# eezkni/UEGAN

Hardware: AMD Instinct MI355X
Metric: train imgs/sec @512px bs=16 on 1/2/4/8 MI355X; infer ms/img (higher is better)
Workload: dtype bf16; 1 GPU; FiveK-shaped 512x512 batch=16/GPU, full G/D/VGG train step (trainer.py:77-119), conv_dim=32, seeded stand-in VGG19; global_batch=16, parallelism=dp1, pool_size=50, collective=none (1 rank), passes=batched (fused.py)

## Files before the change

### include/uegan_hip.h

```cpp
#ifndef UEGAN_HIP_H_
#define UEGAN_HIP_H_

#include <stddef.h>
#include <stdint.h>

#ifdef __cplusplus
extern "C" {
#endif

#define UEGAN_VERSION 105

enum { UEGAN_OK = 0, UEGAN_E_INVALID = -1, UEGAN_E_HIP = -2, UEGAN_E_UNSUPPORTED = -3 };
enum { UEGAN_F32 = 0, UEGAN_BF16 = 1 };
enum { UEGAN_PAD_ZERO = 0, UEGAN_PAD_REFLECT = 1 };
enum { UEGAN_ACT_NONE = 0, UEGAN_ACT_LRELU = 1, UEGAN_ACT_RELU = 2, UEGAN_ACT_TANH = 3,
       UEGAN_ACT_SIGMOID = 4,
       UEGAN_ACT_SWISH = 5, UEGAN_ACT_SELU = 6 };
enum { UEGAN_IMPL_AUTO = 0, UEGAN_IMPL_MFMA = 1, UEGAN_IMPL_DIRECT = 2, UEGAN_IMPL_MFMA_REGSTAGE = 3, UEGAN_IMPL_MFMA_GENERIC = 4 };

typedef void* uegan_stream_t;

int uegan_version(void);
const char* uegan_last_error(void);
int uegan_set_conv_impl(int impl);
enum {
  UEGAN_TUNE_SMALL_GRID = 0,
  UEGAN_TUNE_FOLD_MAX = 1,
  UEGAN_TUNE_HEADS_NO_CG = 2,
  UEGAN_TUNE_WIDE_MIN_GRID = 3,
  UEGAN_TUNE_TALL_MIN_GRID = 4,
  UEGAN_TUNE_TALL_RPW = 5,
  UEGAN_TUNE_TALL_REFLECT = 6,
  UEGAN_TUNE_FLAT_S2 = 7,
  UEGAN_TUNE_TOEP_HEADS = 8,
  UEGAN_TUNE_HEADS_MFMA = 9,
  UEGAN_TUNE_FWD_STATS = 10,
  UEGAN_TUNE_WGRAD_XCD = 11,
  UEGAN_TUNE_VGG_EPI = 12,
  UEGAN_TUNE_GAM_BWD = 13,
  UEGAN_TUNE_COUNT = 14
};
int uegan_set_tuning(int knob, int value, int* previous);
int uegan_selftest_mfma(void* scratch_4096_floats, uegan_stream_t stream);

typedef struct {
  char name[96];
  int64_t launches;
  double total_ms;
  double total_flops;
  double total_bytes;
} uegan_profile_entry;
int uegan_profile_begin(int max_records);
int uegan_profile_end(uegan_profile_entry* out, int max_entries, int* n_entries);

typedef struct {
  int32_t dtype;
  int32_t B, H, W;
  int32_t C1, C2;
  int32_t Ho, Wo, Cout;
  int32_t KH, KW, stride, pad;
  int32_t pad_mode;
  int32_t act;
  int32_t Cin_w, Cout_w;
  int32_t Cin_total;
  int32_t scale_group;
} uegan_conv_desc;

int64_t uegan_packed_k(int64_t k);
int uegan_pack_weights(int dtype, const float* w_oihw, int Cout, int Cin, int KH, int KW, int Cout_pad, int Cin_pad, void* w_ohwi,
                       void* w_ihwo, uegan_stream_t stream);
int uegan_pack_weights_slice(int dtype, const float* w_oihw, int Cout, int Cin, int Cin_total, int KH, int KW, int Cout_pad, int Cin_pad,
                             void* w_ohwi, void* w_ihwo, uegan_stream_t stream);
int uegan_pack_weights_pair(int dtype, const float* w_oihw, int Cout, int Cin, int Cin_total, int KH, int KW, int Cout_pad, int Cin_pad,
                            void* w_ohwi, void* w_ihwo, void* w_ohwi_lo, int dup_cin, uegan_stream_t stream);
typedef struct uegan_pack_entry {
  const float* w_oihw;
  void* w_ohwi;
  void* w_ihwo;
  int64_t start;
  int32_t Cout, Cin, Cin_total, KH, KW, Cout_pad, Cin_pad, Kp, Kp2;
  int32_t flags;
  void* w_ohwi_lo;
} uegan_pack_entry;
int uegan_pack_weights_multi(int dtype, const uegan_pack_entry* table_dev, int n_entries, int64_t total, uegan_stream_t stream);
int uegan_conv2d_fwd(const uegan_conv_desc* d, const void* x1, const void* x2, const void* w_ohwi, const float* bias,
                     const float* scale, void* y, uegan_stream_t stream);
size_t uegan_conv2d_fwd_splitk_workspace_bytes(const uegan_conv_desc* d);
int uegan_conv2d_fwd_splitk(const uegan_conv_desc* d, const void* x1, const void* x2, const void* w_ohwi, const float* bias, const float* scale, void* y,
                            void* workspace, size_t workspace_bytes, uegan_stream_t stream);
size_t uegan_conv2d_fwd_stats_workspace_bytes(const uegan_conv_desc* d);
int uegan_conv2d_fwd_stats(const uegan_conv_desc* d, const void* x1, const void* x2, const void* w_ohwi, const float* bias, const float* scale, void* y,
                           float* mean, float* rstd, float eps, void* workspace, size_t workspace_bytes, int* produced, uegan_stream_t stream);
int uegan_instnorm_apply(int dtype, const void* x, void* y, const float* mean, const float* rstd, int B, int HW, int C, uegan_stream_t stream);

typedef struct {
  const void* x1_lo;
  const void* x2_lo;
  const void* w_lo;
  void* y_lo;
  const void* mul;
  const void* mul_lo;
  void* y_mul;
  void* y_mul_lo;
  const float* res_x;
  const float* res_x2;
  float* res_out;
  float* res_out2;
  float* mean;
  float* rstd;
  void* stats_workspace;
  size_t stats_workspace_bytes;
  float eps;
  int32_t res_split;
  int32_t w_interleaved;
  int32_t reserved;
} uegan_conv_ex;
size_t uegan_conv2d_fwd_ex_workspace_bytes(const uegan_conv_desc* d, const uegan_conv_ex* ex);
int uegan_conv2d_fwd_ex(const uegan_conv_desc* d, const uegan_conv_ex* ex, const void* x1, const void* x2, const void* w_ohwi, const float* bias,
                        const float* scale, void* y, int* taken, uegan_stream_t stream);
int uegan_nchw_to_nhwc_pair(int dtype, const float* x, void* y, int B, int C, int Cp, int H, int W, const float* a, const float* b,
                            uegan_stream_t stream);
int uegan_instnorm_apply_pair(int dtype, const void* x, const void* x_lo, void* y, void* y_lo, const float* mean, const float* rstd, int B, int HW,
                              int C, uegan_stream_t stream);
// ... 210 lines not shown
```

### uegan_amd/csrc/conv_core.h

```cpp
#pragma once
#include "common.h"
#include "conv_internal.h"

#include <stdio.h>
#include <stdlib.h>
#include <utility>
#include <vector>

namespace uegan {

struct ProfRecord {
  hipEvent_t start, stop;
  int kernel_id;
  double flops, bytes;
};
extern bool g_prof_on;
extern std::vector<ProfRecord> g_prof_records;
extern std::vector<std::pair<hipEvent_t, hipEvent_t>> g_prof_pool;
extern size_t g_prof_used;

static inline int prof_key(int kind, bool bf16, int bn, int ks, int mode, int th, bool glds) {
  return (kind << 28) | ((bf16 ? 1 : 0) << 24) | (bn << 12) | (ks << 8) | (mode << 4) | ((th == 32 ? 2 : (th == 16 ? 1 : (th == 4 ? 3 : 0))) << 1) | (glds ? 1 : 0);
}
static void prof_kernel_name(int key, char* buf, size_t n) {
  const int kind = (key >> 28) & 7, bn = (key >> 12) & 0xfff, ks = (key >> 8) & 15, mode = (key >> 4) & 15;
  const char* dt = ((key >> 24) & 1) ? "bf16" : "f32";
  if (kind == 0) snprintf(buf, n, "conv_gemm_kernel<%s,BN=%d,%s>", dt, bn, (key & 1) ? "glds" : "regstage");
  else if (kind == 1) snprintf(buf, n, "conv_patch_kernel<%s,BN=%d,KS=%d,MODE=%d,TH=%d>", dt, bn, ks, mode, 8 << ((key >> 1) & 3));
  else if (kind == 4) snprintf(buf, n, "conv_stream_kernel<%s,TN=%d,PF=%d,MODE=%d>", dt, bn, ks, mode);
  else if (kind == 5) snprintf(buf, n, "conv_s2fwd_kernel<%s,BN=%d,K=%d,TH=%d>", dt, bn, ks, 8 << ((key >> 1) & 3));
  else if (kind == 6) snprintf(buf, n, "conv_toep_kernel<%s,K=%d,MODE=%d>", dt, ks, mode);
  else if (kind == 7 && ((key >> 1) & 3) == 1) snprintf(buf, n, "conv_tall_kernel<%s,BN=%d,KS=%d,MODE=%d%s>", dt, bn, ks, mode, (key & 1) ? "" : ",POOL");
  else if (kind == 7 && ((key >> 1) & 3) == 3) snprintf(buf, n, "conv_flat_kernel<%s,BN=%d,KS=%d>", dt, bn, ks);
  else if (kind == 7) snprintf(buf, n, "conv_wide_kernel<%s,BN=%d,KS=%d,MODE=%d>", dt, bn, ks, mode);
  else if (kind == 3) snprintf(buf, n, "wgrad_tr_kernel<%s,TN=%d,TM=%d%s>", dt, bn, ks, (key & 1) ? ",big" : "");
  else snprintf(buf, n, "conv_wgrad_kernel<%s,BN=%d>", dt, bn);
}

struct ProfScope {
  bool on;
  hipStream_t s;
  ProfRecord rec;
  ProfScope(int kernel_id, double flops, hipStream_t stream, double bytes = 0.0) : on(g_prof_on && g_prof_used < g_prof_pool.size()), s(stream) {
    if (!on) return;
    rec.bytes = bytes;
    rec.start = g_prof_pool[g_prof_used].first;
    rec.stop = g_prof_pool[g_prof_used].second;
    ++g_prof_used;
    rec.kernel_id = kernel_id;
    rec.flops = flops;
    (void)hipEventRecord(rec.start, s);
  }
  ~ProfScope() {
    if (!on) return;
    (void)hipEventRecord(rec.stop, s);
    g_prof_records.push_back(rec);
  }
};

#ifdef UEGAN_HALF_FP16
typedef _Float16 bf16x8_t __attribute__((ext_vector_type(8)));
__device__ __forceinline__ f32x4 mfma_bf16(u32x4 a, u32x4 b, f32x4 c) {
  return __builtin_amdgcn_mfma_f32_16x16x32_f16(__builtin_bit_cast(bf16x8_t, a), __builtin_bit_cast(bf16x8_t, b), c, 0, 0, 0);
}
#else
typedef __bf16 bf16x8_t __attribute__((ext_vector_type(8)));

__device__ __forceinline__ f32x4 mfma_bf16(u32x4 a, u32x4 b, f32x4 c) {
  return __builtin_amdgcn_mfma_f32_16x16x32_bf16(__builtin_bit_cast(bf16x8_t, a), __builtin_bit_cast(bf16x8_t, b), c, 0, 0, 0);
}
#endif
__device__ __forceinline__ f32x4 mfma_f32(float a, float b, f32x4 c) {
  return __builtin_amdgcn_mfma_f32_16x16x4f32(a, b, c, 0, 0, 0);
}

template <typename T> __device__ __forceinline__ u32x4 add_frag(u32x4 a, u32x4 b);
template <> __device__ __forceinline__ u32x4 add_frag<bf16_t>(u32x4 a, u32x4 b) {
  u32x4 r;
#pragma unroll
  for (int d = 0; d < 4; ++d) r[d] = pack_bf16x2(half_lo_to_f32(a[d]) + half_lo_to_f32(b[d]), half_hi_to_f32(a[d]) + half_hi_to_f32(b[d]));
  return r;
}
template <> __device__ __forceinline__ u32x4 add_frag<float>(u32x4 a, u32x4 b) {
  u32x4 r;
#pragma unroll
  for (int d = 0; d < 4; ++d) r[d] = f32_to_bits(bits_to_f32(a[d]) + bits_to_f32(b[d]));
  return r;
}

template <typename T> struct Mma;
template <> struct Mma<bf16_t> {
  static constexpr int NCHUNK = 1;
  static __device__ __forceinline__ void step(const u32x4* a, const u32x4* b, f32x4& acc) { acc = mfma_bf16(a[0], b[0], acc); }
};
template <> struct Mma<float> {
  static constexpr int NCHUNK = 2;
  static __device__ __forceinline__ void step(const u32x4* a, const u32x4* b, f32x4& acc) {
#pragma unroll
    for (int c = 0; c < 2; ++c) {
      acc = mfma_f32(bits_to_f32(a[c].x), bits_to_f32(b[c].x), acc);
      acc = mfma_f32(bits_to_f32(a[c].y), bits_to_f32(b[c].y), acc);
      acc = mfma_f32(bits_to_f32(a[c].z), bits_to_f32(b[c].z), acc);
      acc = mfma_f32(bits_to_f32(a[c].w), bits_to_f32(b[c].w), acc);
    }
  }
};

struct ConvGeom {
  int B, IH, IW;
  int C1, C2, C;
  int OH, OW;
  int KH, KW, stride, pad, pad_mode;
  int mode;
};

__device__ __forceinline__ int src_coord(const ConvGeom& g, int o, int t, int img, int in_n, int out_n) {
  if (g.mode == 0) {
// ... 86 lines not shown
  int N, Kp, act, nbias;
  int nty, ntx;
  int frame;
  int fy0, fy1, fx0, fx1;
  const void* mask;
  int mask_act;
  void* pool_out = nullptr;
  int pool_done = 0;
  void* pool_idx = nullptr;
  int n_idx = 0;
  int n_full = 1 << 30;
  int xcd_map = 0;
  int epi = 0;
  const void* epi_y = nullptr;
  const float* epi_st = nullptr;
  const float* epi_tot = nullptr;
  const float* epi_gscale = nullptr;
  float epi_weight = 0.f;
  const unsigned char* epi_idx = nullptr;
  int rect_y0 = 0, rect_y1 = 0, rect_x0 = 0, rect_x1 = 0;
  int border_only = 0;
  float* stats_part = nullptr;
  int stats_tpi = 0;
  const void* in1_lo = nullptr;
  const void* in2_lo = nullptr;
  const void* w_lo = nullptr;
  void* out_lo = nullptr;
  const void* mul = nullptr;
  const void* mul_lo = nullptr;
  void* out_mul = nullptr;
  void* out_mul_lo = nullptr;
  int src_wrap = 0;
  const float* res_x = nullptr;
  const float* res_x2 = nullptr;
  float* res_out = nullptr;
  float* res_out2 = nullptr;
  int res_split = 1 << 30;
  float* kws = nullptr;
  size_t kws_bytes = 0;
  int kparts = 0, kchunks = 0;
};

static inline int splitk_parts(const ConvArgs& a, int blocks, int nchunk, int* kchunks) {
  *kchunks = nchunk;
  if (!a.kws || a.g.mode != 0 || a.frame || a.out2 || a.mask || a.pool_out || a.stats_part || a.out_lo || a.mul || a.res_out || blocks <= 0) return 1;
  int parts = 1;
  while (parts * 2 <= nchunk && blocks * parts * 2 <= 256) parts *= 2;
  const size_t out_bytes = (size_t)a.g.B * a.g.OH * a.g.OW * a.N * sizeof(float);
  while (parts > 1 && (size_t)parts * out_bytes > a.kws_bytes) parts >>= 1;
  if (parts < 2) return 1;
  *kchunks = (nchunk + parts - 1) / parts;
  return (nchunk + *kchunks - 1) / *kchunks;
}

int splitk_reduce_launch(const ConvArgs& a, hipStream_t s);


constexpr int CONV_TH = 8, CONV_TW = 16, CONV_BM = CONV_TH * CONV_TW;
constexpr int CONV_ROWB = 128;

struct ConvImpl { int impl; bool glds, patch, heads, wgtr, stream; };
extern ConvImpl g_impl;

int check_desc(const uegan_conv_desc* d);
ConvGeom fwd_geom(const uegan_conv_desc* d);
static inline int cin_w(const uegan_conv_desc* d) { return d->Cin_w ? d->Cin_w : d->C1 + d->C2; }
static inline int cin_row(const uegan_conv_desc* d) { return d->Cin_total ? d->Cin_total : cin_w(d); }
static inline int cout_w(const uegan_conv_desc* d) { return d->Cout_w ? d->Cout_w : d->Cout; }
int conv_gemm_run(ConvArgs& a, int dtype, hipStream_t s);
int conv_patch_bf16_a(ConvArgs& a, hipStream_t s, int ks);
int conv_patch_bf16_b(ConvArgs& a, hipStream_t s, int ks);
int conv_patch_f32_a(ConvArgs& a, hipStream_t s, int ks);
int conv_patch_f32_b(ConvArgs& a, hipStream_t s, int ks);
int conv_toep_run(ConvArgs& a, int dtype, hipStream_t s);
bool conv_toep_takes(const ConvArgs& a, int dtype);
bool heads_dgrad_mfma_applicable(const uegan_conv_desc* d);
int heads_dgrad_mfma(const uegan_conv_desc* d, const void* dz, const void* w_ohwi, void* out, hipStream_t s);
int conv_wide_run(ConvArgs& a, int dtype, hipStream_t s, bool interior = false);
int conv_tall_run(ConvArgs& a, int dtype, hipStream_t s, bool interior = false);
int conv_interior_run(ConvArgs& a, int dtype, hipStream_t s);
int conv_s2fwd_run(ConvArgs& a, int dtype, hipStream_t s);
bool conv_flat_applicable(const uegan_conv_desc* d);
int conv_flat_run(const uegan_conv_desc* d, const void* dz, const void* w_ihwo, const float* scale, void* out, hipStream_t s);
int launch_dgrad_images(ConvArgs& a, int dtype, hipStream_t s, bool rows_only);

}
```

### uegan_amd/csrc/runtime.hip

```cpp
#include "conv_core.h"

#include <stdarg.h>

namespace uegan {

static thread_local char g_err[512] = "";

void set_error(const char* fmt, ...) {
  va_list ap;
  va_start(ap, fmt);
  vsnprintf(g_err, sizeof(g_err), fmt, ap);
  va_end(ap);
}

ConvImpl g_impl = {UEGAN_IMPL_AUTO, true, true, true, true, true};
int g_tuning[UEGAN_TUNE_COUNT] = {256, -1, 0, 192, 192, 0, 1, 1, 1, 1, 1, 1, 1, 1};
int g_abl_stream = 0, g_abl_wide = 0;
#ifdef UEGAN_TOOLS_BUILD
extern "C" int uegan_tools_set_ablation(int stream_wgrad_bits, int wide_variant) {
  g_abl_stream = stream_wgrad_bits;
  g_abl_wide = wide_variant;
  return UEGAN_OK;
}
#endif

bool g_prof_on = false;
std::vector<ProfRecord> g_prof_records;
std::vector<std::pair<hipEvent_t, hipEvent_t>> g_prof_pool;
size_t g_prof_used = 0;

__global__ void selftest_mfma_kernel(float* out) {
  const int lane = threadIdx.x & 63;
  f32x4 acc = {0.f, 0.f, 0.f, 0.f};
  const int ai = lane & 15, ak = lane >> 4;
  acc = mfma_f32(ai == ak ? 1.f : 0.f, 100.f * (lane >> 4) + (lane & 15), acc);
  for (int r = 0; r < 4; ++r) out[lane * 4 + r] = acc[r];
  __attribute__((aligned(16))) unsigned short av[8];
  __attribute__((aligned(16))) unsigned short bv[8];
  for (int e = 0; e < 8; ++e) {
    const int k = 8 * (lane >> 4) + e;
    av[e] = f32_to_bf16((lane & 15) == k ? 1.f : 0.f);
    bv[e] = f32_to_bf16((float)(k * 8 + (lane & 15)) * 0.5f);
  }
  f32x4 acc2 = {0.f, 0.f, 0.f, 0.f};
  acc2 = mfma_bf16(*reinterpret_cast<u32x4*>(av), *reinterpret_cast<u32x4*>(bv), acc2);
  for (int r = 0; r < 4; ++r) out[256 + lane * 4 + r] = acc2[r];
  typedef float f32x16_t __attribute__((ext_vector_type(16)));
  __attribute__((aligned(16))) unsigned short bk[8];
  for (int e = 0; e < 8; ++e) {
    const int k = 8 * (lane >> 5) + e;
    av[e] = f32_to_bf16((lane & 31) == k ? 1.f : 0.f);
    bk[e] = f32_to_bf16((float)(k + 1));
    bv[e] = f32_to_bf16((float)((lane & 31) + 1));
  }
  f32x16_t z16;
  for (int r = 0; r < 16; ++r) z16[r] = 0.f;
  const bf16x8_t a8 = __builtin_bit_cast(bf16x8_t, *reinterpret_cast<u32x4*>(av));
#ifdef UEGAN_HALF_FP16
  const f32x16_t d1 = __builtin_amdgcn_mfma_f32_32x32x16_f16(a8, __builtin_bit_cast(bf16x8_t, *reinterpret_cast<u32x4*>(bk)), z16, 0, 0, 0);
  const f32x16_t d2 = __builtin_amdgcn_mfma_f32_32x32x16_f16(a8, __builtin_bit_cast(bf16x8_t, *reinterpret_cast<u32x4*>(bv)), z16, 0, 0, 0);
#else
  const f32x16_t d1 = __builtin_amdgcn_mfma_f32_32x32x16_bf16(a8, __builtin_bit_cast(bf16x8_t, *reinterpret_cast<u32x4*>(bk)), z16, 0, 0, 0);
  const f32x16_t d2 = __builtin_amdgcn_mfma_f32_32x32x16_bf16(a8, __builtin_bit_cast(bf16x8_t, *reinterpret_cast<u32x4*>(bv)), z16, 0, 0, 0);
#endif
  for (int r = 0; r < 16; ++r) {
    out[512 + lane * 16 + r] = d1[r];
    out[1536 + lane * 16 + r] = d2[r];
  }
}

}

using namespace uegan;

extern "C" int uegan_version(void) { return UEGAN_VERSION; }
extern "C" const char* uegan_last_error(void) { return g_err; }

extern "C" int uegan_set_tuning(int knob, int value, int* previous) {
  UEGAN_CHECK_ARG(knob >= 0 && knob < UEGAN_TUNE_COUNT, "unknown tuning knob %d", knob);
  if (previous) *previous = g_tuning[knob];
  g_tuning[knob] = value;
  return UEGAN_OK;
}

extern "C" int uegan_set_conv_impl(int impl) {
  const int old = g_impl.impl;
  g_impl = {impl, true, true, true, true, true};
  if (impl == UEGAN_IMPL_MFMA_REGSTAGE) { g_impl.impl = UEGAN_IMPL_MFMA; g_impl.glds = false; g_impl.heads = false; g_impl.wgtr = false; }
  else if (impl == UEGAN_IMPL_MFMA_GENERIC) { g_impl.impl = UEGAN_IMPL_MFMA; g_impl.patch = false; g_impl.heads = false; g_impl.wgtr = false; g_impl.stream = false; }
  return old;
}

extern "C" int uegan_selftest_mfma(void* scratch, uegan_stream_t stream) {
  UEGAN_CHECK_ARG(scratch, "null scratch");
  hipLaunchKernelGGL(selftest_mfma_kernel, dim3(1), dim3(64), 0, (hipStream_t)stream, (float*)scratch);
  UEGAN_CHECK_LAUNCH();
  return UEGAN_OK;
}

// ... 45 lines not shown
```

### uegan_amd/csrc/wgrad.hip

```cpp
#include "conv_core.h"

namespace uegan {

struct WgradArgs {
  ConvGeom g;
  const void* in1;
  const void* in2;
  const void* dz;
  float* ws;
  int N, zC, ktot;
  int WS, WSlog, R;
  int nxb, nyb;
  int steps_total, steps_per_split;
};

constexpr int WG_BK = 128;

__device__ __forceinline__ void transpose_chunks(const u32x4 (&in)[4], u32x4 (&out)[4]) {
  out[0] = u32x4{in[0].x, in[1].x, in[2].x, in[3].x};
  out[1] = u32x4{in[0].y, in[1].y, in[2].y, in[3].y};
  out[2] = u32x4{in[0].z, in[1].z, in[2].z, in[3].z};
  out[3] = u32x4{in[0].w, in[1].w, in[2].w, in[3].w};
}
__device__ __forceinline__ void transpose_chunks(const u32x4 (&in)[8], u32x4 (&out)[8]) {
// ... 218 lines not shown
  for (int ch0 = 0; ch0 < nch; ch0 += cp) {
    const int ch = ch0 + c_lane;
    float s[V];
#pragma unroll
    for (int e = 0; e < V; ++e) s[e] = 0.f;
    if (ch < nch)
      for (size_t p = (size_t)blockIdx.x * rows + r_lane; p < npix; p += (size_t)gridDim.x * rows) {
        float v[V];
        Vec<T, V>::ld(dz + p * zC + ch * V, v);
#pragma unroll
        for (int e = 0; e < V; ++e) s[e] += v[e];
      }
#pragma unroll
    for (int e = 0; e < V; ++e) red[e][threadIdx.x] = s[e];
    __syncthreads();
    for (int half = rows >> 1; half > 0; half >>= 1) {
      if (r_lane < half) {
#pragma unroll
        for (int e = 0; e < V; ++e) red[e][threadIdx.x] += red[e][threadIdx.x + half * cp];
      }
      __syncthreads();
    }
    if (r_lane == 0 && ch < nch) {
#pragma unroll
      for (int e = 0; e < V; ++e) part[(size_t)blockIdx.x * zC + ch * V + e] = red[e][c_lane];
    }
    __syncthreads();
  }
}
__global__ void bias_grad_final_kernel(const float* part, float* dbias, int nblocks, int C, int zC, int acc) {
  __shared__ float red[16];
  const int c = blockIdx.x;
  float s = 0.f;
  for (int k = threadIdx.x; k < nblocks; k += blockDim.x) s += part[(size_t)k * zC + c];
  s = block_sum(s, red);
  if (threadIdx.x == 0) dbias[c] = s + (acc ? dbias[c] : 0.f);
}

template <typename T>
__global__ void wgrad_direct_kernel(WgradArgs a, float* dw, const float* scale_p, int Cin_w, int accum, int Cin_row) {
  const ConvGeom& g = a.g;
  const T* in1 = static_cast<const T*>(a.in1);
  const T* in2 = static_cast<const T*>(a.in2);
  const T* dz = static_cast<const T*>(a.dz);
  const size_t total = (size_t)a.N * a.ktot;
  const float scale = scale_p ? *scale_p : 1.f;
  for (size_t idx = (size_t)blockIdx.x * blockDim.x + threadIdx.x; idx < total; idx += (size_t)gridDim.x * blockDim.x) {
    const int n = (int)(idx / a.ktot), kk = (int)(idx - (size_t)n * a.ktot);
    const int tap = kk / g.C, c = kk - tap * g.C, ty = tap / g.KW, tx = tap - ty * g.KW;
    if (c >= Cin_w) continue;
    float acc = 0.f;
    for (int b = 0; b < g.B; ++b)
      for (int oy = 0; oy < g.OH; ++oy) {
        const int sy = src_coord(g, oy, ty, 0, g.IH, g.OH);
        if (sy < 0) continue;
        for (int ox = 0; ox < g.OW; ++ox) {
          const int sx = src_coord(g, ox, tx, 0, g.IW, g.OW);
          if (sx < 0) continue;
          const size_t pix = ((size_t)b * g.IH + sy) * g.IW + sx;
          const float xv = (c < g.C1) ? DT<T>::ld(in1 + pix * g.C1 + c) : DT<T>::ld(in2 + pix * g.C2 + (c - g.C1));
          acc += xv * DT<T>::ld(dz + (((size_t)b * g.OH + oy) * g.OW + ox) * a.zC + n);
        }
      }
    float* o = dw + ((size_t)n * Cin_row + c) * (g.KH * g.KW) + tap;
    *o = acc * scale + (accum ? *o : 0.f);
  }
}

}

using namespace uegan;

int uegan::wgrad_reduce_1x1(const float* ws, float* dw, int nsplit, int N, int C, int Cin_w, int Cin_row, size_t pstride, int acc, hipStream_t s) {
  const size_t total = (size_t)N * C;
  hipLaunchKernelGGL(wgrad_reduce_kernel, dim3((unsigned)((total + 31) / 32)), dim3(256), 0, s, ws, dw, (float*)nullptr, (const float*)nullptr, nsplit, N, C,
                     Cin_w, 1, 1, pstride, acc, 0, Cin_row);
  UEGAN_CHECK_LAUNCH();
  return UEGAN_OK;
}

struct WgradPlan {
  WgradArgs a;
  WgradTrPlan tr;
  int nsplit, bn;
  dim3 grid;
  size_t ws_bytes;
};

static void wgrad_plan(const uegan_conv_desc* d, WgradPlan& p) {
  WgradArgs& a = p.a;
  a.g = fwd_geom(d);
  a.N = cout_w(d);
  a.zC = d->Cout;
  a.ktot = d->KH * d->KW * (d->C1 + d->C2);
  auto done = [&](int bn, int nsplit, dim3 grid) {
    p.bn = bn; p.nsplit = nsplit; p.grid = grid;
    p.ws_bytes = ((size_t)nsplit * ((size_t)a.N * a.ktot + a.N) + (size_t)BIAS_BLOCKS * d->Cout) * sizeof(float);
  };
  if (g_impl.impl != UEGAN_IMPL_DIRECT && wgtr_plan(d, a.g, p.tr)) return done(-1, p.tr.nsplit_eff, p.tr.grid);
  const int npix = d->dtype == UEGAN_BF16 ? 64 : 32;
  int ws = 1, wl = 0;
  while (ws < d->Wo && ws < npix) { ws <<= 1; ++wl; }
  a.WS = ws; a.WSlog = wl; a.R = npix / ws;
  a.nxb = (d->Wo + ws - 1) / ws;
  a.nyb = (d->Ho + a.R - 1) / a.R;
  a.steps_total = d->B * a.nyb * a.nxb;
  if (g_impl.impl != UEGAN_IMPL_DIRECT && g_impl.heads && heads_applicable(d)) {
    const int nb = heads_wgrad_blocks(d);
    return done(0, nb, dim3(nb));
  }
  const int bn = a.N <= 16 ? 16 : (a.N <= 32 ? 32 : (a.N <= 64 ? 64 : 128));
  const int tiles = ((a.ktot + WG_BK - 1) / WG_BK) * ((a.N + bn - 1) / bn);
  int want = (1536 + tiles - 1) / tiles;
  if (want < 1) want = 1;
  if (want > a.steps_total) want = a.steps_total;
  a.steps_per_split = (a.steps_total + want - 1) / want;
  const int nsplit = (a.steps_total + a.steps_per_split - 1) / a.steps_per_split;
  done(bn, nsplit, dim3((a.ktot + WG_BK - 1) / WG_BK, (a.N + bn - 1) / bn, nsplit));
}

extern "C" size_t uegan_conv2d_wgrad_workspace_bytes(const uegan_conv_desc* d) {
  if (check_desc(d)) return 0;
  WgradPlan p;
  wgrad_plan(d, p);
  return p.ws_bytes;
}

template <typename T>
static int run_wgrad(const uegan_conv_desc* d, WgradPlan& p, const float* scale, float* dw, float* dbias, int accmask, hipStream_t s) {
  WgradArgs& a = p.a;
  const int acc = accmask & 1, accb = (accmask >> 1) & 1;
  const double flops = 2.0 * (double)d->B * d->Ho * d->Wo * a.N * (double)a.ktot, elems = (double)d->B * d->H * d->W * (d->C1 + d->C2) + (double)d->B * d->Ho * d->Wo * d->Cout;
  auto reduce = [&](bool bias_too) {
    const size_t nw = (size_t)a.N * a.ktot, total = nw + (bias_too ? a.N : 0);
    hipLaunchKernelGGL(wgrad_reduce_kernel, dim3((unsigned)((total + 31) / 32)), dim3(256), 0, s, a.ws, dw, bias_too ? dbias : (float*)nullptr, scale, p.nsplit,
                       a.N, a.g.C, cin_w(d), a.g.KH, a.g.KW, p.bn == -1 ? (size_t)p.tr.a.pstride : nw, acc, accb, cin_row(d));
  };
  if (g_impl.impl == UEGAN_IMPL_DIRECT) {
    const size_t total = (size_t)a.N * a.ktot;
    const int blocks = (int)((total + 255) / 256 < 4096 ? (total + 255) / 256 : 4096);
    hipLaunchKernelGGL((wgrad_direct_kernel<T>), dim3(blocks), dim3(256), 0, s, a, dw, scale, cin_w(d), acc, cin_row(d));
  } else if (p.bn == -1) {
    WgradTrPlan& tr = p.tr;
    tr.a.in1 = a.in1; tr.a.in2 = a.in2; tr.a.dz = a.dz; tr.a.ws = a.ws;
    tr.a.want_bias = dbias ? 1 : 0;
    {
      ProfScope prof(prof_key(3, true, tr.tn, tr.tm, 0, 8, tr.big), flops, s, 2.0 * elems);
      wgtr_launch(tr, s);
      UEGAN_CHECK_LAUNCH();
    }
    reduce(dbias != nullptr);
    UEGAN_CHECK_LAUNCH();
    return UEGAN_OK;
  } else if (p.bn == 0) {
    int rc = heads_wgrad(d, a.in1, a.dz, a.ws, s);
    if (rc) return rc;
    reduce(false);
  } else {
    {
      ProfScope prof(prof_key(2, DT<T>::kDtype == UEGAN_BF16, p.bn, 0, 0, 8, false), flops, s, sizeof(T) * elems);
      if (p.bn == 128) hipLaunchKernelGGL((conv_wgrad_kernel<T, 128>), p.grid, dim3(256), 0, s, a);
      else if (p.bn == 64) hipLaunchKernelGGL((conv_wgrad_kernel<T, 64>), p.grid, dim3(256), 0, s, a);
      else if (p.bn == 32) hipLaunchKernelGGL((conv_wgrad_kernel<T, 32>), p.grid, dim3(256), 0, s, a);
      else hipLaunchKernelGGL((conv_wgrad_kernel<T, 16>), p.grid, dim3(256), 0, s, a);
      UEGAN_CHECK_LAUNCH();
    }
    reduce(false);
  }
  UEGAN_CHECK_LAUNCH();
  if (dbias) {
    const size_t npix = (size_t)d->B * d->Ho * d->Wo;
    const int nch = a.zC / DT<T>::EPC;
    int cp = 1;
    while (cp < nch && cp < 64) cp <<= 1;
    const size_t rows = 256 / cp;
    size_t blocks = (npix + rows * 8 - 1) / (rows * 8);
    if (blocks > BIAS_BLOCKS) blocks = BIAS_BLOCKS;
    if (blocks < 1) blocks = 1;
    float* part = a.ws + (size_t)p.nsplit * a.N * a.ktot;
    hipLaunchKernelGGL((bias_grad_partial_kernel<T>), dim3((unsigned)blocks), dim3(256), 0, s, static_cast<const T*>(a.dz), part, npix, a.zC);
    UEGAN_CHECK_LAUNCH();
    hipLaunchKernelGGL(bias_grad_final_kernel, dim3(a.N), dim3(256), 0, s, part, dbias, (int)blocks, a.N, a.zC, accb);
    UEGAN_CHECK_LAUNCH();
  }
  return UEGAN_OK;
}

extern "C" int uegan_conv2d_wgrad(const uegan_conv_desc* d, const void* x1, const void* x2, const void* dz, const float* scale,
                                  float* dw_oihw, float* dbias, void* workspace, size_t workspace_bytes, uegan_stream_t stream) {
  return uegan_conv2d_wgrad_acc(d, x1, x2, dz, scale, dw_oihw, dbias, workspace, workspace_bytes, 0, stream);
}

extern "C" int uegan_conv2d_wgrad_acc(const uegan_conv_desc* d, const void* x1, const void* x2, const void* dz, const float* scale,
                                      float* dw_oihw, float* dbias, void* workspace, size_t workspace_bytes, int accumulate,
                                      uegan_stream_t stream) {
  int rc = check_desc(d);
  if (rc) return rc;
  UEGAN_CHECK_ARG(x1 && dz && dw_oihw && (d->C2 == 0 || x2), "null pointer");
  WgradPlan p;
  wgrad_plan(d, p);
  UEGAN_CHECK_ARG(workspace && workspace_bytes >= p.ws_bytes, "wgrad workspace too small: %zu < %zu", workspace_bytes, p.ws_bytes);
  p.a.in1 = x1; p.a.in2 = d->C2 ? x2 : x1; p.a.dz = dz; p.a.ws = static_cast<float*>(workspace);
  hipStream_t s = (hipStream_t)stream;
  UEGAN_CHECK_ARG(accumulate >= 0 && accumulate <= 3, "accumulate is a bit mask: 1 = dw, 2 = dbias");
  return d->dtype == UEGAN_F32 ? run_wgrad<float>(d, p, scale, dw_oihw, dbias, accumulate, s) : run_wgrad<bf16_t>(d, p, scale, dw_oihw, dbias, accumulate, s);
}
```

Before: 503.2 imgs/sec.

## Add Toeplitz-style MFMA weight-gradient kernel for 7x7 thin-channel convs

Adds a dedicated weight-gradient kernel for 7x7 stride-1 convolutions whose output or input side has three real channels (32->3 and 8->32 shapes, such as the generator's head and stem layers). It stages a tile of the 32-channel tensor and a 3-channel plane into double-buffered LDS, then treats the 49 taps times 3 channels as MFMA columns so one thick-tile read feeds every tap. The default on path also computes the bias gradient, either inside the kernel or with a small extra reduction. It replaces the general transposed wgrad path for these layers, and adds some workspace and planning complexity.

```diff
diff --git a/include/uegan_hip.h b/include/uegan_hip.h
--- a/include/uegan_hip.h
+++ b/include/uegan_hip.h
@@ -38,7 +38,8 @@
   UEGAN_TUNE_WGRAD_XCD = 11,
   UEGAN_TUNE_VGG_EPI = 12,
   UEGAN_TUNE_GAM_BWD = 13,
-  UEGAN_TUNE_COUNT = 14
+  UEGAN_TUNE_WGRAD_TOEP = 14,
+  UEGAN_TUNE_COUNT = 15
 };
 int uegan_set_tuning(int knob, int value, int* previous);
 int uegan_selftest_mfma(void* scratch_4096_floats, uegan_stream_t stream);
diff --git a/uegan_amd/csrc/conv_core.h b/uegan_amd/csrc/conv_core.h
--- a/uegan_amd/csrc/conv_core.h
+++ b/uegan_amd/csrc/conv_core.h
@@ -33,6 +33,7 @@
   else if (kind == 7 && ((key >> 1) & 3) == 1) snprintf(buf, n, "conv_tall_kernel<%s,BN=%d,KS=%d,MODE=%d%s>", dt, bn, ks, mode, (key & 1) ? "" : ",POOL");
   else if (kind == 7 && ((key >> 1) & 3) == 3) snprintf(buf, n, "conv_flat_kernel<%s,BN=%d,KS=%d>", dt, bn, ks);
   else if (kind == 7) snprintf(buf, n, "conv_wide_kernel<%s,BN=%d,KS=%d,MODE=%d>", dt, bn, ks, mode);
+  else if (kind == 3 && bn == 0xfff) snprintf(buf, n, "wgrad_toep_kernel<%s,%s>", dt, mode ? "B" : "A");
   else if (kind == 3) snprintf(buf, n, "wgrad_tr_kernel<%s,TN=%d,TM=%d%s>", dt, bn, ks, (key & 1) ? ",big" : "");
   else snprintf(buf, n, "conv_wgrad_kernel<%s,BN=%d>", dt, bn);
 }
@@ -285,6 +286,14 @@
 int conv_s2fwd_run(ConvArgs& a, int dtype, hipStream_t s);
 bool conv_flat_applicable(const uegan_conv_desc* d);
 int conv_flat_run(const uegan_conv_desc* d, const void* dz, const void* w_ihwo, const float* scale, void* out, hipStream_t s);
+constexpr int WGRAD_TOEP_MIN_H = 32, WGRAD_TOEP_MIN_W = 32;
+struct WgradToepPlan {
+  bool case_b;
+  int tiles_x, tiles_y, tiles_total, tiles_per_block, blocks;
+};
+bool wgrad_toep_takes(const uegan_conv_desc* d);
+bool wgrad_toep_plan(const uegan_conv_desc* d, WgradToepPlan& p);
+int wgrad_toep_launch(const uegan_conv_desc* d, const WgradToepPlan& p, const void* x, const void* dz, float* ws, bool want_bias, hipStream_t s);
 int launch_dgrad_images(ConvArgs& a, int dtype, hipStream_t s, bool rows_only);
 
 }
diff --git a/uegan_amd/csrc/runtime.hip b/uegan_amd/csrc/runtime.hip
--- a/uegan_amd/csrc/runtime.hip
+++ b/uegan_amd/csrc/runtime.hip
@@ -14,7 +14,7 @@
 }
 
 ConvImpl g_impl = {UEGAN_IMPL_AUTO, true, true, true, true, true};
-int g_tuning[UEGAN_TUNE_COUNT] = {256, -1, 0, 192, 192, 0, 1, 1, 1, 1, 1, 1, 1, 1};
+int g_tuning[UEGAN_TUNE_COUNT] = {256, -1, 0, 192, 192, 0, 1, 1, 1, 1, 1, 1, 1, 1, 1};
 int g_abl_stream = 0, g_abl_wide = 0;
 #ifdef UEGAN_TOOLS_BUILD
 extern "C" int uegan_tools_set_ablation(int stream_wgrad_bits, int wide_variant) {
diff --git a/uegan_amd/csrc/wgrad.hip b/uegan_amd/csrc/wgrad.hip
--- a/uegan_amd/csrc/wgrad.hip
+++ b/uegan_amd/csrc/wgrad.hip
@@ -324,6 +324,7 @@
 struct WgradPlan {
   WgradArgs a;
   WgradTrPlan tr;
+  WgradToepPlan toep;
   int nsplit, bn;
   dim3 grid;
   size_t ws_bytes;
@@ -339,6 +340,11 @@
     p.bn = bn; p.nsplit = nsplit; p.grid = grid;
     p.ws_bytes = ((size_t)nsplit * ((size_t)a.N * a.ktot + a.N) + (size_t)BIAS_BLOCKS * d->Cout) * sizeof(float);
   };
+  if (wgrad_toep_plan(d, p.toep)) {
+    done(-2, p.toep.blocks, dim3(p.toep.blocks));
+    p.ws_bytes += (size_t)p.toep.blocks * 6 * sizeof(float);
+    return;
+  }
   if (g_impl.impl != UEGAN_IMPL_DIRECT && wgtr_plan(d, a.g, p.tr)) return done(-1, p.tr.nsplit_eff, p.tr.grid);
   const int npix = d->dtype == UEGAN_BF16 ? 64 : 32;
   int ws = 1, wl = 0;
@@ -376,12 +382,21 @@
   auto reduce = [&](bool bias_too) {
     const size_t nw = (size_t)a.N * a.ktot, total = nw + (bias_too ? a.N : 0);
     hipLaunchKernelGGL(wgrad_reduce_kernel, dim3((unsigned)((total + 31) / 32)), dim3(256), 0, s, a.ws, dw, bias_too ? dbias : (float*)nullptr, scale, p.nsplit,
-                       a.N, a.g.C, cin_w(d), a.g.KH, a.g.KW, p.bn == -1 ? (size_t)p.tr.a.pstride : nw, acc, accb, cin_row(d));
+                       a.N, a.g.C, cin_w(d), a.g.KH, a.g.KW, p.bn == -1 ? (size_t)p.tr.a.pstride : (p.bn == -2 ? nw + a.N : nw), acc, accb, cin_row(d));
   };
   if (g_impl.impl == UEGAN_IMPL_DIRECT) {
     const size_t total = (size_t)a.N * a.ktot;
     const int blocks = (int)((total + 255) / 256 < 4096 ? (total + 255) / 256 : 4096);
     hipLaunchKernelGGL((wgrad_direct_kernel<T>), dim3(blocks), dim3(256), 0, s, a, dw, scale, cin_w(d), acc, cin_row(d));
+  } else if (p.bn == -2) {
+    {
+      ProfScope prof(prof_key(3, true, 0xfff, 0, p.toep.case_b ? 1 : 0, 8, false), flops, s, 2.0 * elems);
+      const int rc = wgrad_toep_launch(d, p.toep, a.in1, a.dz, a.ws, dbias != nullptr, s);
+      if (rc) return rc;
+    }
+    reduce(dbias != nullptr);
+    UEGAN_CHECK_LAUNCH();
+    return UEGAN_OK;
   } else if (p.bn == -1) {
     WgradTrPlan& tr = p.tr;
     tr.a.in1 = a.in1; tr.a.in2 = a.in2; tr.a.dz = a.dz; tr.a.ws = a.ws;
diff --git a/uegan_amd/csrc/wgrad_toep.hip b/uegan_amd/csrc/wgrad_toep.hip
--- /dev/null
+++ b/uegan_amd/csrc/wgrad_toep.hip
@@ -0,0 +1,324 @@
+#include "conv_core.h"
+
+namespace uegan {
+
+constexpr int WT_TH = 8, WT_TW = 32;
+constexpr int WT_PR = WT_TH + 6;
+constexpr int WT_PD = 19, WT_ROWB = 80;
+constexpr int WT_NT = 3;
+constexpr int WT_COLS = 49 * WT_NT;
+constexpr int WT_PLANEB = WT_PR * WT_ROWB;
+constexpr int WT_THICKB = WT_TH * WT_TW * 64;
+constexpr int WT_BUFB = WT_THICKB + 2 * WT_NT * WT_PLANEB;
+constexpr int WT_ITEMS = WT_PR * WT_PD;
+
+struct WgradToepArgs {
+  const unsigned char* thick;
+  const unsigned char* thin;
+  float* ws;
+  float* bias_part;
+  int B, H, W, reflect;
+  int ktot, pstride, nw;
+  int tiles_x, tiles_y, tiles_total, tiles_per_block;
+};
+
+__device__ __forceinline__ void wt_wait_lds() {
+#ifndef UEGAN_EMU
+  asm volatile("s_waitcnt lgkmcnt(0)" ::: "memory");
+#endif
+}
+
+template <bool CASE_B>
+__global__ void __launch_bounds__(256, 3) wgrad_toep_kernel(WgradToepArgs a) {
+  __shared__ __attribute__((aligned(16))) unsigned char lds[2 * WT_BUFB];
+  __shared__ double red[256];
+  const int tid = threadIdx.x, lane = tid & 63;
+  const int wave = __builtin_amdgcn_readfirstlane(tid >> 6);
+  const int g4 = lane >> 4, sj = (lane & 15) >> 2, seg = lane & 3;
+  const int GH = CASE_B ? a.H : a.H + 6, GW = CASE_B ? a.W : a.W + 6;
+
+  const int c0 = 4 * (g4 & 1) + 16 * (g4 >> 1);
+  int taddr[2];
+#pragma unroll
+  for (int i = 0; i < 2; ++i) {
+    const int r = c0 + sj, ch = 16 * i + 4 * seg;
+    taddr[i] = r * 64 + ((((ch >> 3) ^ wgtr_swz(64, r))) << 4) + ((ch >> 2) & 1) * 8;
+  }
+  int naddr[3];
+  bool ones[3], live[3];
+#pragma unroll
+  for (int m = 0; m < 3; ++m) {
+    const int ct = wave + 4 * m;
+    const int j = ct * 16 + (lane & 15);
+    live[m] = ct * 16 < WT_COLS + (CASE_B ? 1 : 0);
+    ones[m] = CASE_B && j == WT_COLS;
+    const int jj = j < WT_COLS ? j : 0;
+    const int t = jj / WT_NT, n = jj - t * WT_NT, ty = t / 7, tx = t - ty * 7;
+    const int sy = CASE_B ? ty : 6 - ty, sx = CASE_B ? tx : 6 - tx;
+    const int aa = c0 + sx;
+    naddr[m] = WT_THICKB + (((aa & 1) * WT_NT + n) * WT_PR + sy) * WT_ROWB + (aa >> 1) * 4;
+  }
+  const uint32_t one2 = (uint32_t)f32_to_bf16(1.f) * 0x10001u;
+  const u32x4 ones4 = u32x4{one2, one2, one2, one2};
+
+  f32x4 acc[2][3];
+#pragma unroll
+  for (int i = 0; i < 2; ++i)
+#pragma unroll
+    for (int m = 0; m < 3; ++m) acc[i][m] = f32x4{0.f, 0.f, 0.f, 0.f};
+  double bsum[WT_NT] = {0.0, 0.0, 0.0};
+
+  const int t_begin = blockIdx.x * a.tiles_per_block;
+  int t_end = t_begin + a.tiles_per_block;
+  if (t_end > a.tiles_total) t_end = a.tiles_total;
+
+  auto tile_origin = [&](int t, int& b, int& y0, int& x0) {
+    const int txi = t % a.tiles_x, tq = t / a.tiles_x;
+    b = tq / a.tiles_y;
+    y0 = (tq - b * a.tiles_y) * WT_TH;
+    x0 = txi * WT_TW;
+  };
+  auto src_pix = [&](int b, int py, int px) -> long long {
+    int y = py - 3, x = px - 3;
+    if (a.reflect) {
+      y = reflect_idx(y, a.H); x = reflect_idx(x, a.W);
+      y = y < 0 ? 0 : (y >= a.H ? a.H - 1 : y);
+      x = x < 0 ? 0 : (x >= a.W ? a.W - 1 : x);
+    } else if (y < 0 || y >= a.H || x < 0 || x >= a.W) {
+      return -1;
+    }
+    return ((long long)b * a.H + y) * a.W + x;
+  };
+
+  auto stage_thick = [&](int t, int bufi) {
+    int b, y0, x0;
+    tile_origin(t, b, y0, x0);
+    unsigned char* dst = lds + bufi * WT_BUFB;
+    const int kcol = (tid >> 2) & 31, pos = tid & 3;
+#pragma unroll
+    for (int it = 0; it < 4; ++it) {
+      const int krow = 2 * it + (tid >> 7);
+      const int r = krow * WT_TW + kcol;
+      const int q = pos ^ wgtr_swz(64, r);
+      const int gy = y0 + krow, gx = x0 + kcol;
+      const void* src = g_zero16;
+      if (gy < GH && gx < GW) {
+        const long long pix = CASE_B ? ((long long)b * a.H + gy) * a.W + gx : src_pix(b, gy, gx);
+        if (pix >= 0) src = a.thick + pix * 64 + q * 16;
+      }
+      wgtr_glds16(src, dst + (it * 256 + wave * 64) * 16);
+    }
+  };
+  struct Thin { u32x2 p[2][3]; };
+  auto load_thin = [&](int t, Thin& v) {
+    int b, y0, x0;
+    tile_origin(t, b, y0, x0);
+#pragma unroll
+    for (int it = 0; it < 2; ++it) {
+      const int id = it * 256 + tid;
+      const int pr = id / WT_PD, i = id - pr * WT_PD;
+#pragma unroll
+      for (int k = 0; k < 3; ++k) {
+        v.p[it][k] = u32x2{0u, 0u};
+        const int pc = 2 * i + k;
+        if (id >= WT_ITEMS || pc >= WT_TW + 6) continue;
+        long long pix;
+        if (CASE_B) {
+          pix = src_pix(b, y0 + pr, x0 + pc);
+        } else {
+          const int y = y0 - 6 + pr, x = x0 - 6 + pc;
+          pix = (y >= 0 && y < a.H && x >= 0 && x < a.W) ? ((long long)b * a.H + y) * a.W + x : -1;
+        }
+        if (pix >= 0) v.p[it][k] = *reinterpret_cast<const u32x2*>(a.thin + pix * 16);
+      }
+    }
+  };
+  auto write_thin = [&](const Thin& v, int bufi) {
+    unsigned char* pl = lds + bufi * WT_BUFB + WT_THICKB;
+#pragma unroll
+    for (int it = 0; it < 2; ++it) {
+      const int id = it * 256 + tid;
+      if (id >= WT_ITEMS) continue;
+      const int pr = id / WT_PD, i = id - pr * WT_PD;
+      const int o = pr * WT_ROWB + i * 4;
+#pragma unroll
+      for (int n = 0; n < WT_NT; ++n) {
+        uint32_t h[3];
+#pragma unroll
+        for (int k = 0; k < 3; ++k) {
+          const uint32_t word = n < 2 ? v.p[it][k].x : v.p[it][k].y;
+          h[k] = (n & 1) ? (word >> 16) : (word & 0xffffu);
+        }
+        *reinterpret_cast<uint32_t*>(pl + n * WT_PLANEB + o) = h[0] | (h[1] << 16);
+        *reinterpret_cast<uint32_t*>(pl + (WT_NT + n) * WT_PLANEB + o) = h[1] | (h[2] << 16);
+        if (!CASE_B && pr >= 6 && i >= 3) bsum[n] += (double)bf16_to_f32((bf16_t)h[0]) + (double)bf16_to_f32((bf16_t)h[1]);
+      }
+    }
+  };
+
+  Thin nxt;
+  if (t_begin < t_end) {
+    stage_thick(t_begin, 0);
+    load_thin(t_begin, nxt);
+    write_thin(nxt, 0);
+  }
+  for (int t = t_begin; t < t_end; ++t) {
+    const int bufi = (t - t_begin) & 1;
+    wgtr_wait_loads();
+    wt_wait_lds();
+    raw_barrier();
+    if (t + 1 < t_end) {
+      stage_thick(t + 1, bufi ^ 1);
+      load_thin(t + 1, nxt);
+    }
+    const unsigned char* buf = lds + bufi * WT_BUFB;
+    f32x4 half[2][3];
+#pragma unroll
+    for (int hh = 0; hh < 2; ++hh) {
+      const unsigned char* hb = buf + hh * 4 * WT_TW * 64;
+      u32x4 af[4][2];
+#pragma unroll
+      for (int ks = 0; ks < 4; ++ks)
+#pragma unroll
+        for (int i = 0; i < 2; ++i) {
+          const u32x2 lo = lds_read_tr16(hb + ks * WT_TW * 64 + taddr[i]), hi = lds_read_tr16(hb + ks * WT_TW * 64 + taddr[i] + 8 * 64);
+          af[ks][i] = u32x4{lo.x, lo.y, hi.x, hi.y};
+        }
+#pragma unroll
+      for (int m = 0; m < 3; ++m) {
+        if (!live[m]) continue;
+        u32x4 bf[4];
+#pragma unroll
+        for (int ks = 0; ks < 4; ++ks) {
+          const uint32_t* p = reinterpret_cast<const uint32_t*>(buf + naddr[m] + (hh * 4 + ks) * WT_ROWB);
+          bf[ks] = ones[m] ? ones4 : u32x4{p[0], p[1], p[4], p[5]};
+        }
+#pragma unroll
+        for (int i = 0; i < 2; ++i) {
+          f32x4 part[4];
+#pragma unroll
+          for (int ks = 0; ks < 4; ++ks) part[ks] = mfma_bf16(af[ks][i], bf[ks], f32x4{0.f, 0.f, 0.f, 0.f});
+          const f32x4 h4 = (part[0] + part[1]) + (part[2] + part[3]);
+          if (hh == 0) half[i][m] = h4;
+          else acc[i][m] += half[i][m] + h4;
+        }
+      }
+    }
+    __builtin_amdgcn_sched_barrier(0);
+    if (t + 1 < t_end) write_thin(nxt, bufi ^ 1);
+  }
+
+  float* ws = a.ws + (size_t)blockIdx.x * a.pstride;
+#pragma unroll
+  for (int m = 0; m < 3; ++m) {
+    if (!live[m]) continue;
+    const int j = (wave + 4 * m) * 16 + (lane & 15);
+#pragma unroll
+    for (int i = 0; i < 2; ++i)
+#pragma unroll
+      for (int r = 0; r < 4; ++r) {
+        const int row = 16 * i + 4 * g4 + r;
+        if (j < WT_COLS) {
+          const int tt = j / WT_NT, n = j - tt * WT_NT;
+          if (CASE_B) ws[(size_t)row * a.ktot + tt * 8 + n] = acc[i][m][r];
+          else ws[(size_t)n * a.ktot + tt * 32 + row] = acc[i][m][r];
+        } else if (CASE_B && j == WT_COLS) {
+          ws[a.nw + row] = acc[i][m][r];
+        }
+      }
+  }
+  if (!CASE_B) {
+    for (int n = 0; n < WT_NT; ++n) {
+      red[tid] = bsum[n];
+      __syncthreads();
+      for (int h = 128; h > 0; h >>= 1) {
+        if (tid < h) red[tid] += red[tid + h];
+        __syncthreads();
+      }
+      if (tid == 0) {
+        const float hi = (float)red[0];
+        a.bias_part[(blockIdx.x * WT_NT + n) * 2] = hi;
+        a.bias_part[(blockIdx.x * WT_NT + n) * 2 + 1] = (float)(red[0] - (double)hi);
+        ws[a.nw + n] = 0.f;
+      }
+      __syncthreads();
+    }
+  }
+}
+
+__global__ void __launch_bounds__(256) wgrad_toep_bias_kernel(const float* bias_part, float* ws, int nw, int blocks) {
+  __shared__ double red[256];
+  const int tid = threadIdx.x;
+  for (int n = 0; n < WT_NT; ++n) {
+    double s = 0.0;
+    for (int k = tid; k < blocks; k += 256) s += (double)bias_part[(k * WT_NT + n) * 2] + (double)bias_part[(k * WT_NT + n) * 2 + 1];
+    red[tid] = s;
+    __syncthreads();
+    for (int h = 128; h > 0; h >>= 1) {
+      if (tid < h) red[tid] += red[tid + h];
+      __syncthreads();
+    }
+    if (tid == 0) ws[nw + n] = (float)red[0];
+    __syncthreads();
+  }
+}
+
+static int wgrad_toep_blocks() {
+#if defined(UEGAN_EMU)
+  return 8;
+#else
+  return 768;
+#endif
+}
+
+bool wgrad_toep_takes(const uegan_conv_desc* d) {
+  if (g_tuning[UEGAN_TUNE_WGRAD_TOEP] == 0 || d->dtype != UEGAN_BF16 || g_impl.impl == UEGAN_IMPL_DIRECT || !g_impl.wgtr) return false;
+  if (d->KH != 7 || d->KW != 7 || d->stride != 1 || d->pad != 3 || d->C2 != 0 || d->Ho != d->H || d->Wo != d->W) return false;
+  if (d->pad_mode != UEGAN_PAD_REFLECT && d->pad_mode != UEGAN_PAD_ZERO) return false;
+  if (d->H < WGRAD_TOEP_MIN_H || d->W < WGRAD_TOEP_MIN_W) return false;
+  const bool case_a = d->C1 == 32 && d->Cout == 8 && cout_w(d) == WT_NT && cin_w(d) == 32;
+  const bool case_b = d->C1 == 8 && d->Cout == 32 && cout_w(d) == 32 && cin_w(d) == WT_NT;
+  if (!case_a && !case_b) return false;
+  const long long tiles = (long long)d->B * ((d->H + 6 + WT_TH - 1) / WT_TH) * ((d->W + 6 + WT_TW - 1) / WT_TW);
+  return d->B > 0 && tiles < (1 << 30);
+}
+
+bool wgrad_toep_plan(const uegan_conv_desc* d, WgradToepPlan& p) {
+  if (!wgrad_toep_takes(d)) return false;
+  p.case_b = d->C1 == 8;
+  const int GH = p.case_b ? d->H : d->H + 6, GW = p.case_b ? d->W : d->W + 6;
+  p.tiles_x = (GW + WT_TW - 1) / WT_TW;
+  p.tiles_y = (GH + WT_TH - 1) / WT_TH;
+  p.tiles_total = d->B * p.tiles_x * p.tiles_y;
+  const int knob = g_tuning[UEGAN_TUNE_WGRAD_TOEP];
+  int cap = wgrad_toep_blocks();
+  if (knob >= 2 && knob < cap) cap = knob;
+  if (cap > p.tiles_total) cap = p.tiles_total;
+  p.tiles_per_block = (p.tiles_total + cap - 1) / cap;
+  p.blocks = (p.tiles_total + p.tiles_per_block - 1) / p.tiles_per_block;
+  return true;
+}
+
+int wgrad_toep_launch(const uegan_conv_desc* d, const WgradToepPlan& p, const void* x, const void* dz, float* ws, bool want_bias, hipStream_t s) {
+  WgradToepArgs a;
+  a.thick = static_cast<const unsigned char*>(p.case_b ? dz : x);
+  a.thin = static_cast<const unsigned char*>(p.case_b ? x : dz);
+  a.ws = ws;
+  a.B = d->B; a.H = d->H; a.W = d->W;
+  a.reflect = d->pad_mode == UEGAN_PAD_REFLECT ? 1 : 0;
+  a.ktot = 49 * d->C1;
+  a.nw = cout_w(d) * a.ktot;
+  a.pstride = a.nw + cout_w(d);
+  a.tiles_x = p.tiles_x; a.tiles_y = p.tiles_y; a.tiles_total = p.tiles_total; a.tiles_per_block = p.tiles_per_block;
+  a.bias_part = ws + (size_t)p.blocks * a.pstride;
+  if (p.case_b) hipLaunchKernelGGL((wgrad_toep_kernel<true>), dim3(p.blocks), dim3(256), 0, s, a);
+  else hipLaunchKernelGGL((wgrad_toep_kernel<false>), dim3(p.blocks), dim3(256), 0, s, a);
+  UEGAN_CHECK_LAUNCH();
+  if (!p.case_b && want_bias) {
+    hipLaunchKernelGGL(wgrad_toep_bias_kernel, dim3(1), dim3(256), 0, s, a.bias_part, ws, a.nw, p.blocks);
+    UEGAN_CHECK_LAUNCH();
+  }
+  return UEGAN_OK;
+}
+
+}
```

Result: no change. 506.3 imgs/sec (median of 6 runs) (+0.6%).
